# jayHuggie/PathTracer_CUDA_Interactive

Measured on AMD Instinct MI355X. Metric: Msamples/sec (rays x spp x bounces = intersect() calls per second), scenes/cbox/cbox.xml 640x480 spp=64, higher is better.
Workload: dtype f32

## Files before the change

pathtracer_cuda_interactive_amd/csrc/pt_api.hip:

```cpp
#include <cmath>
#include <cstdio>
#include <cstdlib>
#include <cstring>
#include <initializer_list>
#include <iterator>
#include <limits>
#include <mutex>
#include <type_traits>

#include "pt_scene.h"
#include "pt_transform.h"
#include "pt_denoise.h"
#include "pt_gradient.h"
#include "pt_temporal.h"
#include "pt_kernels.h"
#include "pt_kernel_q.h"
#include "pt_query.h"

using namespace ptk;

static thread_local std::string g_err;
int pt_fail(int code, const std::string& msg) { g_err = msg; return code; }
static int fail(int code, const std::string& msg) { return pt_fail(code, msg); }

// ... 84 lines not shown
    bool lds_scene() const { return res == 1 || res == 2; }
};

int choose_trace(const pt_scene* S, int traversal, bool nee, bool listed, TraceChoice* out) {
    TraceChoice c{};
    c.which = which_tree(S);
    c.res = scene_residency(S, c.which);
    const bool exact = traversal == PT_TRAVERSAL_EXACT;
    if (nee && (S->opt_kernel < 2 || !exact))
        return fail(PT_ERR_UNSUPPORTED, "PT_RENDER_NEE runs on the default kernel with exact traversal only");
    c.family = S->opt_kernel == 1 ? 1 : (S->opt_kernel == 3 && !nee && exact && !listed) ? 3 : 2;
    c.prune = !exact; c.stats = S->opt_stats != 0; c.nee = nee; c.list = listed;
    c.postpone = c.family == 3 && !c.lds_scene() && c.which == 1;
    c.spec = !(S->tri_only && S->opt_specialize) ? 0 : (S->diffuse_only ? 2 : 1);
    if (nee && c.spec == 1) c.spec = 0;
    if (c.family == 2)
        c.sched = v2_schedule((nee || listed) ? V2Schedule{0, 0, 6} : V2Schedule{(int)S->opt_v2_thresh, (int)S->opt_v2_inner, (int)S->opt_v2_minw},
                              c.lds_scene(), c.which == 1 && !nee);
    const pt_scene::Tree& T = S->tree[c.which];
    c.reg_stack = S->opt_reg_stack && c.family == 2 && !nee && !listed && c.spec == 2 && !S->opt_v2_thresh && !S->opt_v2_inner &&
                  (c.sched.minw == 5 || c.sched.minw == 6) &&
                  reg_stack_on(c.res, c.sched.thresh, c.sched.inner, c.which == 1, T.stack_cap - 1, T.num_nodes, S->dev.num_prims);
    c.sweep = S->opt_leaf_sweep && leaf_sweep_on(c.reg_stack, exact, c.stats, c.res, S->dev.num_prims, (int)S->sweep.count) &&
              S->sweep_tab.p && sweep_layout_fits(S->sweep.count, (uint32_t)S->dev.num_prims, (uint32_t)T.num_nodes, kLdsNodeStride);
    c.block_threads = c.family == 3 ? kQBlock : kBlock;
    c.feed_waves = c.family == 3 ? kQS : kBlock / 64;
    c.redo_lanes = c.family == 3 ? kQS * 64 : kBlock;
    *out = c;
    return PT_OK;
}

LdsPlan make_plan(const pt_scene* S, const TraceChoice& c) {
    LdsPlan lp{};
    const pt_scene::Tree& T = S->tree[c.which];
    uint32_t off = 0;
    if (c.res == 3) {
        const uint32_t stack_bytes = (uint32_t)(kBlock / 64) * (uint32_t)T.stack_cap * 64u * 4u;
        const uint32_t budget = S->opt_lds_budget_kb > 0 ? (uint32_t)S->opt_lds_budget_kb * 1024u : kTopLdsBudget;
        const uint32_t room = budget > stack_bytes ? budget - stack_bytes : 0u;
        lp.top_count = std::min<uint32_t>(T.top_avail, room / (uint32_t)sizeof(DNode));
        lp.nodes_off = 0;
        off = lp.top_count * (uint32_t)sizeof(DNode);
    } else if (c.res != 0) {
        lp.nodes_off = off;
        off = align16(off + (c.res == 2 ? 8u * oct_table_pitch((uint32_t)T.num_nodes, kLdsNodeStride)
                                        : (uint32_t)T.num_nodes * kLdsNodeStride));
        lp.prims_off = off; off = align16(off + (uint32_t)S->dev.num_prims * sizeof(DPrim));
// ... 122 lines not shown
        if (kV2Schedules[k].thresh == c.sched.thresh && kV2Schedules[k].inner == c.sched.inner && kV2Schedules[k].minw == c.sched.minw) si = k;
    return among<0, 1, 2, 3, 4, 5, 6, 7, 8>(si, [&](auto SI) { return among<0, 1, 2, 3>(c.res, [&](auto R) {
           return among<false, true>(c.nee, [&](auto N) { return among<false, true>(c.list, [&](auto LI) {
           static constexpr V2Schedule s = kV2Schedules[PT_CONST(SI)];
           if constexpr (!v2_compiled(PT_CONST(R), false, s, 0, PT_CONST(N), PT_CONST(LI))) return TraceEntry{};
           else return among<0, 1, 2>(c.spec, [&](auto SP) { return among<false, true>(c.prune, [&](auto P) {
           return among<false, true>(c.stats, [&](auto S) {
               if constexpr (v2_compiled(PT_CONST(R), PT_CONST(P), s, PT_CONST(SP), PT_CONST(N), PT_CONST(LI)))
                   return v2k<PT_CONST(R), PT_CONST(P), PT_CONST(S), s.thresh, s.inner, s.minw, PT_CONST(SP), PT_CONST(N), PT_CONST(LI)>();
               else return TraceEntry{}; }); }); }); }); }); }); });
}
#undef PT_CONST

void launch_trace(const pt_scene* S, const TraceChoice& c, const TraceEntry& e, int grid, hipStream_t stream, const RenderDev& rd,
                  const LdsPlan& lp, const QParams& qp, float4* samples) {
    void* const fn = const_cast<void*>(e.fn);
    if (c.family == 3)
        hipLaunchKernelGGL(reinterpret_cast<TraceFnQ>(fn), dim3(grid), dim3(c.block_threads), lp.total, stream, S->dev, rd, lp, qp,
                           samples, S->work_counter(), S->counters());
    else if (c.sweep) {
        const SweepClasses cls = S->sweep_classes_now();
        hipLaunchKernelGGL(reinterpret_cast<SweepFn>(fn), dim3(grid), dim3(c.block_threads), lp.total, stream, S->dev, rd, lp,
                           samples, S->work_counter(), S->counters(),
                           SweepLayoutDev{S->sweep_tab_now(), S->sweep.count, sweep_classes_pitch(cls), cls.pairs, cls.fam});
    } else
        hipLaunchKernelGGL(reinterpret_cast<TraceFn>(fn), dim3(grid), dim3(c.block_threads), lp.total, stream, S->dev, rd, lp,
                           samples, S->work_counter(), S->counters());
}

int read_slot_sums(const pt_scene* S, unsigned long long* out) {
    std::vector<unsigned long long> raw(kTimelineBase);
    HIP_TRY(hipMemcpy(raw.data(), S->counters(), raw.size() * sizeof(unsigned long long), hipMemcpyDeviceToHost));
    std::fill(out, out + kSlotStride, 0ull);
    for (int s = 0; s < kCounterSlots; s++)
        for (int k = 0; k < kSlotStride; k++) out[k] += raw[(size_t)s * kSlotStride + k];
    return PT_OK;
}

int launch_grid(int num_cus, int blocks_per_cu, uint64_t work_items, int block_threads = kBlock) {
    const uint64_t blocks_needed = (work_items + (uint64_t)block_threads - 1) / (uint64_t)block_threads;
    return (int)std::max<uint64_t>(1, std::min<uint64_t>((uint64_t)num_cus * (uint64_t)blocks_per_cu, blocks_needed));
}

struct RowSel {
    int begin, step, count;
};

// ... 1193 lines not shown
    else if (k == "lds_budget_kb") S->opt_lds_budget_kb = value;
    else if (k == "chunk") S->opt_chunk = value;
    else if (k == "item_order") S->opt_item_order = value;
    else if (k == "specialize") S->opt_specialize = value;
    else if (k == "timing_frames") {
        if (value < 0 || value > 4096) return fail(PT_ERR_INVALID_ARG, "timing_frames must be 0 .. 4096");
        S->opt_timing_frames = value;
    }
    else if (k == "kernel") { if (value < 1 || value > 3) return fail(PT_ERR_INVALID_ARG, "kernel must be 1, 2 or 3"); S->opt_kernel = value; }
    else if (k == "frames_in_flight") {
        if (value < 1 || value > kMaxFramesInFlight) return fail(PT_ERR_INVALID_ARG, "frames_in_flight must be 1 .. " + std::to_string(kMaxFramesInFlight));
        S->opt_frames_in_flight = value;
    }
    else if (k == "q_target") S->opt_q_target = value;
    else if (k == "q_swap") S->opt_q_swap = value;
    else if (k == "q_low") S->opt_q_low = value;
    else if (k == "v2_thresh") S->opt_v2_thresh = value;
    else if (k == "v2_inner") S->opt_v2_inner = value;
    else if (k == "v2_minw") S->opt_v2_minw = value;
    else if (k == "reg_stack") { if (value != 0 && value != 1) return fail(PT_ERR_INVALID_ARG, "reg_stack must be 0 or 1"); S->opt_reg_stack = value; }
    else if (k == "leaf_sweep") { if (value != 0 && value != 1) return fail(PT_ERR_INVALID_ARG, "leaf_sweep must be 0 or 1"); S->opt_leaf_sweep = value; }
    else if (k == "sweep_pairs") { if (value != 0 && value != 1) return fail(PT_ERR_INVALID_ARG, "sweep_pairs must be 0 or 1"); S->opt_sweep_pairs = value; }
    else if (k == "sweep_families") { if (value != 0 && value != 1) return fail(PT_ERR_INVALID_ARG, "sweep_families must be 0 or 1"); S->opt_sweep_families = value; }
    else if (k == "query_refill") { if (value < 0 || value > 64) return fail(PT_ERR_INVALID_ARG, "query_refill must be 0 (automatic) .. 64"); S->opt_query_refill = value; }
    else if (k == "query_guides") { if (value < 0 || value > 2) return fail(PT_ERR_INVALID_ARG, "query_guides must be 0 (automatic), 1 or 2"); S->opt_query_guides = value; }
    else if (k == "query_blocks") { if (value < 0 || value > 4096) return fail(PT_ERR_INVALID_ARG, "query_blocks must be 0 (automatic) .. 4096"); S->opt_query_blocks = value; }
    else if (k == "tree_cost" || k == "rebuild_at_permille") {
        if (k == "tree_cost" && value != 0 && value != 1) return fail(PT_ERR_INVALID_ARG, "tree_cost must be 0 or 1");
        if (k == "rebuild_at_permille" && value != 0 && value < 1001) return fail(PT_ERR_INVALID_ARG, "rebuild_at_permille must be 0 (never) or at least 1001");
        const bool was_on = S->cost_on();
        (k == "tree_cost" ? S->opt_tree_cost : S->opt_rebuild_at) = value;
        if (!was_on && S->cost_on()) S->cost_forget();
    }
    else return fail(PT_ERR_INVALID_ARG, "unknown option " + k);
    return PT_OK;
}

int pt_scene_get_info(pt_scene* S, const char* key, int64_t* value) {
    if (!S || !key || !value) return fail(PT_ERR_INVALID_ARG, "null argument");
    const std::string k(key);
    TraceChoice next;
    (void)choose_trace(S, k == "vgprs_pruned" ? PT_TRAVERSAL_PRUNED : PT_TRAVERSAL_EXACT, false, false, &next);
    DeviceGuard guard;
    unsigned long long c[kSlotStride];
    if (k == "grid") *value = S->info_grid;
    else if (k == "lds_bytes") *value = S->info_lds_bytes;
// ... 42 lines not shown
        const int t = k[9] - '0';
        *value = (S->cost_on() && (t == 0 || S->have_fast)) ? cost_permille(S, t) : 1000;
    }
    else if (k == "refit_shape0" || k == "refit_shape1") {
        const ptf::Plan& pl = S->refit_plan[k[11] - '0'];
        *value = !pl.built ? 0 : pl.whole_tree ? 1 : pl.narrow_top < pl.levels - 1 ? 2 : 3;
    }
    else if (k == "kernel") *value = S->info_kernel;
    else if (k == "trace_variant") *value = S->info_trace_variant;
    else if (k == "path_bank") *value = S->info_path_bank;
    else if (k == "leaf_sweep") *value = S->info_leaf_sweep;
    else if (k == "sweep_boxes") *value = S->sweep_groups;
    else if (k.rfind("sweep_share_pairs", 0) == 0 || k.rfind("sweep_flat_pairs", 0) == 0 || k == "sweep_general_pairs") {
        const SweepClasses c = S->sweep_classes_now();
        const bool flat = k[6] == 'f';
        const std::string axis = k.substr(flat ? 16 : 17);
        if (k == "sweep_general_pairs") *value = c.pairs.general;
        else if (axis.empty()) *value = sweep_classes_sharing(c, flat, -1);
        else if (axis == "_x" || axis == "_y" || axis == "_z") *value = sweep_classes_sharing(c, flat, axis[1] - 'x');
        else return fail(PT_ERR_INVALID_ARG, "unknown info key " + k);
    }
    else if (k == "sweep_pair2_records") *value = sweep_pair2_records(S->sweep_classes_now().fam);
    else if (k == "sweep_valu_model") *value = sweep_valu_model(S->sweep_classes_now());
    else if (k == "reg_stack") *value = S->info_reg_stack;
    else if (k == "block_threads") *value = S->info_kernel == 3 ? kQBlock : kBlock;
    else if (k == "frames_in_flight") *value = S->opt_frames_in_flight;
    else if (k == "query_chunk") *value = ptq::kQueryChunk;
    else if (k == "query_guides") *value = S->info_query_guides;
    else if (k == "query_grid") *value = S->info_query_grid;
    else if (k.rfind("qdiag", 0) == 0 && k.size() >= 6 && k.size() <= 7 && k.find_first_not_of("0123456789", 5) == std::string::npos &&
             std::stoi(k.substr(5)) < 11) {
        int rc = synced_slot_sums(S, guard, c);
        if (rc) return rc;
        *value = (int64_t)c[4 + std::stoi(k.substr(5))];
    }
    else if (k.rfind("diag", 0) == 0 && k.size() >= 5 && k.size() <= 7 && k.find_first_not_of("0123456789", 4) == std::string::npos &&
             std::stoi(k.substr(4)) < 8 + kNumCounters - kTimelineBase) {
        unsigned long long v = 0;
        const int idx = std::stoi(k.substr(4));
        if (idx < 8) {
            int rc = synced_slot_sums(S, guard, c);
            if (rc) return rc;
            v = c[4 + idx];
        } else {
            if (int grc = guard.enter(S->device)) return grc;
            HIP_TRY(hipStreamSynchronize(S->last_stream));
// ... 113 lines not shown
```

pathtracer_cuda_interactive_amd/csrc/pt_kernels.h:

```cpp
#pragma once

#include <hip/hip_runtime.h>

#include <type_traits>

#include "pt_layout.h"
#include "pt_leaf_sweep.h"
#include "pt_math.h"
#include "pt_path_bank.h"
#include "pt_path_index.h"
#include "pt_sweep_layout.h"
#include "pt_sweep_families.h"
#include "pt_sweep_pairs.h"
#include "pt_temporal.h"
#include "pt_trace.h"

namespace ptk {

using namespace ptl;


#ifndef PT_BLOCK
#define PT_BLOCK 256
#endif
constexpr int kBlock = PT_BLOCK;
constexpr uint32_t kMaxChunk = 256;

__device__ __forceinline__ uint32_t lane_rank(unsigned long long mask) {
    return __builtin_amdgcn_mbcnt_hi((uint32_t)(mask >> 32), __builtin_amdgcn_mbcnt_lo((uint32_t)mask, 0u));
}

__device__ __forceinline__ unsigned long long wave_sum(unsigned long long v) {
    for (int off = 32; off > 0; off >>= 1) v += __shfl_down(v, off, 64);
    return v;
}
// ... 251 lines not shown

template <int RES, bool PRUNE, bool STATS, int MINW>
__global__ __launch_bounds__(kBlock, (kBlock > 256 ? 1 : MINW)) void trace_kernel_v2_reg(SceneDev scn, RenderDev rp, LdsPlan lp,
                                                              float4* __restrict__ samples,
                                                              uint32_t* __restrict__ work_counter,
                                                              unsigned long long* __restrict__ counters) {
    constexpr int THRESH = 40, INNER = 162, SPEC = 2;
    constexpr bool NEE = false, LIST = false, REG = true;
#include "pt_trace_v2_body.h"
}

#ifndef PT_SWEEP_LEAF_STEPS
#define PT_SWEEP_LEAF_STEPS 4
#endif
#ifndef PT_SWEEP_THRESH
#define PT_SWEEP_THRESH 48
#endif
struct SweepLayoutDev {
    const unsigned char* tab;
    uint32_t groups;
    uint32_t box_pitch;
    SweepPairClasses classes;
    SweepFamilyClasses fam;
};
struct SweepKernelArgs {
    SceneDev scn; RenderDev rp; LdsPlan lp; float4* samples; uint32_t* work_counter; unsigned long long* counters; SweepLayoutDev sweep;
};
static_assert(offsetof(SweepKernelArgs, rp) == offsetof(TraceKernelArgs, rp), "reload_render_args reads rp at TraceKernelArgs' offset");
static_assert(offsetof(SweepLayoutDev, fam) + 16 <= sizeof(SweepLayoutDev), "step (3) reads the three PAIR2 count words as one load of four: the fourth must lie inside the argument");

__device__ __forceinline__ ptd::SceneView make_sweep_view(const SceneDev& scn, const LdsPlan& lp, const SweepLayoutDev& sweep,
                                                          unsigned char* smem) {
    const uint32_t slots_off = sweep_slots_off(sweep.groups);
    stage_to_lds(smem + lp.nodes_off, sweep.tab, slots_off);
    const DPrim* gslots = reinterpret_cast<const DPrim*>(sweep.tab + slots_off);
    DPrim* lslots = reinterpret_cast<DPrim*>(smem + lp.nodes_off + slots_off);
    for (uint32_t i = threadIdx.x; i < (uint32_t)scn.num_prims; i += blockDim.x) {
        const float4 a = ptd::ld4(gslots + i, 0), b = ptd::ld4(gslots + i, 1), c = ptd::ld4(gslots + i, 2);
        DPrim g;
        g.v[0] = a.x; g.v[1] = a.y; g.v[2] = a.z; g.v[3] = a.w; g.v[4] = b.x; g.v[5] = b.y; g.v[6] = b.z; g.v[7] = b.w; g.v[8] = c.x;
        g.info = __builtin_bit_cast(int32_t, c.y); g.light = __builtin_bit_cast(int32_t, c.z); g.pad = __builtin_bit_cast(int32_t, c.w);
        const DPrim r = sweep_stage_record(g);
        float4* d = reinterpret_cast<float4*>(lslots + i);
        d[0] = make_float4(r.v[0], r.v[1], r.v[2], r.v[3]);
        d[1] = make_float4(r.v[4], r.v[5], r.v[6], r.v[7]);
        d[2] = make_float4(r.v[8], c.y, c.z, c.w);
    }
    stage_to_lds(smem + lp.prims_off, scn.prims, (uint32_t)scn.num_prims * sizeof(DPrim));
    stage_to_lds(smem + lp.normals_off, scn.normals, (uint32_t)scn.num_prims * sizeof(DNormals));
    stage_to_lds(smem + lp.mats_off, scn.materials, (uint32_t)scn.num_materials * sizeof(DMaterial));
    stage_to_lds(smem + lp.emis_off, scn.emission, (uint32_t)scn.num_emission * sizeof(DEmission));
    __syncthreads();
    ptd::SceneView sv;
    sv.top_nodes = nullptr;
    sv.top_count = 0;
    sv.nodes = reinterpret_cast<const DNode*>(smem + lp.nodes_off);
    sv.prims = reinterpret_cast<const DPrim*>(smem + lp.prims_off);
    sv.normals = reinterpret_cast<const DNormals*>(smem + lp.normals_off);
    sv.materials = reinterpret_cast<const DMaterial*>(smem + lp.mats_off);
    sv.emission = reinterpret_cast<const DEmission*>(smem + lp.emis_off);
    sv.node_stride = kLdsNodeStride;
    sv.oct_stride = sweep.box_pitch;
    sv.lights = scn.lights;
    sv.num_emission = scn.num_emission;
    sv.root_ref = scn.root_ref;
    sv.fixed_order = scn.fixed_order;
    sv.ref_nodes = scn.ref_nodes; sv.ref_path = scn.ref_path; sv.ref_anc = scn.ref_anc; sv.ref_levels = scn.ref_levels;
    sv.bg = ptm::mk(scn.bg[0], scn.bg[1], scn.bg[2]);
    return sv;
}
// ... 399 lines not shown
```

pathtracer_cuda_interactive_amd/csrc/pt_scene.h:

```cpp
#pragma once
#include <hip/hip_runtime.h>

#include <algorithm>
#include <chrono>
#include <cstdint>
#include <string>
#include <utility>
#include <vector>

#include "../../include/pt_api.h"
#include "pt_internal.h"
#include "pt_layout.h"
#include "pt_leaf_sweep.h"
#include "pt_sweep_families.h"
#include "pt_sweep_pairs.h"
#include "pt_scene_refit.h"

#define HIP_TRY(expr)                                                                              \
    do {                                                                                           \
        hipError_t e_ = (expr);                                                                    \
        if (e_ != hipSuccess)                                                                      \
            return pt_fail(e_ == hipErrorNoDevice ? PT_ERR_NO_DEVICE : PT_ERR_DEVICE,              \
                           std::string(#expr) + ": " + hipGetErrorString(e_));                     \
    } while (0)

#define ENTER_DEVICE(S) DeviceGuard guard; if (int grc_ = guard.enter((S)->device)) return grc_

namespace ptkc {
constexpr int kBlock = 256, kCounterStride = 32, kQueryRing = 64, kLdsNodeStride = 64;
}

using namespace ptl;

template <class T>
struct DevBuf {
    T* p = nullptr;
    size_t n = 0;
// ... 176 lines not shown
    int64_t opt_top_cache = 1;
    int64_t opt_fast_tree = 1;
    int64_t opt_chunk = 0;
    int64_t opt_lds_budget_kb = 0;
    int64_t opt_item_order = 1;
    int64_t opt_xcd_regions = 0;
    int64_t opt_kernel = 2;
    int64_t opt_q_target = 0, opt_q_swap = 0, opt_q_low = 0;
    int64_t opt_v2_thresh = 0, opt_v2_inner = 0, opt_v2_minw = 0;
    int64_t opt_reg_stack = 1;
    int64_t opt_leaf_sweep = 1;
    int64_t opt_sweep_pairs = 1;
    int64_t opt_sweep_families = 1;
    SweepTable sweep{};
    int sweep_groups = 0;
    DevBuf<unsigned char> sweep_tab;
    DevBuf<unsigned char> sweep_tab_pairs[2];
    SweepClasses sweep_classes[2] = {};
    SweepClasses sweep_classes_now() const {
        if (!sweep.count) return SweepClasses{};
        return opt_sweep_pairs && sweep_tab_pairs[opt_sweep_families].p ? sweep_classes[opt_sweep_families] : sweep_classes_of_pairs(sweep_pairs_none(sweep.count));
    }
    const unsigned char* sweep_tab_now() const { return opt_sweep_pairs && sweep_tab_pairs[opt_sweep_families].p ? sweep_tab_pairs[opt_sweep_families].p : sweep_tab.p; }
    int64_t create_us[7] = {0, 0, 0, 0, 0, 0, 0}, sweep_on_device = 0;
    int64_t info_grid = 0, info_lds_bytes = 0, info_lds_scene = 0, info_passes = 0, info_occupancy = 0, info_blocks_per_cu = 0, info_debug_reruns = 0, fast_cost_permille = 0, info_kernel = 0, info_trace_variant = 0, info_path_bank = 0, info_reg_stack = 0, info_leaf_sweep = 0;
    struct PassEvents { hipEvent_t t0, t1, r0, r1; };
    struct FrameRec { std::vector<PassEvents> ev; size_t passes = 0; };
    std::vector<FrameRec> frames;
    uint64_t frame_seq = 0;
    int64_t opt_timing_frames = 1;
    const FrameRec* last_frame() const { return frame_seq && !frames.empty() ? &frames[(frame_seq - 1) % frames.size()] : nullptr; }
    void drop_events() {
        for (auto& f : frames)
            for (auto& pe : f.ev) { (void)hipEventDestroy(pe.t0); (void)hipEventDestroy(pe.t1); (void)hipEventDestroy(pe.r0); (void)hipEventDestroy(pe.r1); }
        frames.clear();
        frame_seq = 0;
    }
    const void* cfg_fn = nullptr;
    uint32_t cfg_lds = 0;
    int cfg_occ = 0;
    ~pt_scene() {
        drop_query();
        for (auto& T : tree) { T.nodes.release(); T.nodes_oct.release(); }
        drop_slots(); drop_events();
        prims.release(); normals.release(); materials.release(); emission.release(); lights.release();
        for (auto& pl : refit_plan) ptf::plan_release(&pl);
// ... 31 lines not shown
```

pathtracer_cuda_interactive_amd/csrc/pt_scene_life.hip:

```cpp
#include <cmath>
#include <cstdlib>
#include <cstring>
#include <exception>
#include <limits>
#include <queue>

#include "pt_scene.h"
#include "pt_tree_sweep.h"
#include "pt_sweep_build.h"
#include "pt_scene_prep.h"
#include "pt_tree_cost.h"
#include "pt_scene_transform.h"
#include "pt_transform.h"
#include "pt_sweep_layout.h"
#include "pt_sweep_families.h"
#include "pt_sweep_pairs.h"

namespace {
using namespace ptkc;

constexpr uint32_t kOctNodeLimit = 24 * 1024;
constexpr int kMaxStack = 64;
constexpr int kMinInternalTree = 16;
constexpr int kDeviceSweepMin = 4096;
#ifndef PT_TOP_NODES
#define PT_TOP_NODES 512
#endif
constexpr uint32_t kTopNodes = PT_TOP_NODES;
constexpr uint32_t kMaxLdsBudget = 160 * 1024;

bool prepared_on_device(int N) {
    const char* v = std::getenv("PT_SWEEP_BUILD");
    return N >= kDeviceSweepMin && !(v && std::string(v) == "host");
}

struct TreeHost {
    std::vector<DNode> nodes;
    int32_t root_ref = 0;
// ... 270 lines not shown
    int32_t froot = 0, fdepth = 0;
    bool ok = true, fnested = true;
    try {
        pts::build_sweep_tree(boxes_host, N, fnodes, &froot, &fdepth);
    } catch (const std::exception&) {
        ok = false;
    }
    built(try_device);
    c.ok = ok && convert_tree(fnodes.data(), (int)fnodes.size(), froot, N, c.host, nullptr, &fnested, true) == PT_OK && fnested;
    return c;
}

void drop_internal_tree(pt_scene* S, const char* why) {
    S->have_fast = S->fast_is_callers_topology = false;
    S->no_fast_why = why;
    S->tree[1].nodes.release(); S->tree[1].nodes_oct.release(); S->tree[1].have_oct = false;
    S->ref_path.release(); S->ref_anc.release();
}

int64_t probe_permille(const unsigned long long v[2]) { return v[0] ? (int64_t)((1000ull * v[1] + v[0] / 2) / v[0]) : 1000; }
bool probe_wins(const unsigned long long v[2]) { return v[1] * 100ull < v[0] * 90ull; }

int make_sweep_tables(const TreeHost& fast, const DPrim* prims, int N, SweepTable& sweep, int& sweep_groups, DevBuf<unsigned char>& sweep_tab,
                      DevBuf<unsigned char> (&sweep_tab_pairs)[2], SweepClasses (&classes)[2]) {
    sweep = SweepTable{};
    sweep_groups = 0;
    for (SweepClasses& c : classes) c = SweepClasses{};
    SweepGroup groups[kSweepMaxPrims];
    const int n = build_sweep_groups(fast.nodes.data(), (int)fast.nodes.size(), N, kLdsNodeStride, groups);
    if (n > 0) {
        sweep_groups = n;
        std::vector<unsigned char> tab(n <= kSweepMaxBoxes ? sweep_layout_bytes((uint32_t)n, (uint32_t)N) : 0);
        SweepGroup paired[kSweepMaxBoxes];
        int perm[kSweepMaxBoxes];
        SweepClasses cls[2] = {};
        std::vector<unsigned char> tab_pairs[2];
        const DNode* nodes = fast.nodes.data();
        const int num_nodes = (int)fast.nodes.size();
        bool ok = n <= kSweepMaxBoxes && build_sweep_layout(groups, n, nodes, num_nodes, kLdsNodeStride, prims, N, tab.data());
        for (int m = 0; ok && m < 2; m++) {
            tab_pairs[m].resize(tab.size());
            ok = build_sweep_families(groups, n, nodes, num_nodes, kLdsNodeStride, m, paired, perm, &cls[m]) &&
                 build_sweep_layout(paired, n, nodes, num_nodes, kLdsNodeStride, prims, N, tab_pairs[m].data()) &&
                 build_sweep_family_tables(paired, n, cls[m], nodes, num_nodes, kLdsNodeStride, tab_pairs[m].data());
        }
        if (ok && !(sweep_stream_fits(sweep_classes_of_pairs(sweep_pairs_none((uint32_t)n)), (uint32_t)n, (uint32_t)N) &&
                    sweep_stream_fits(cls[0], (uint32_t)n, (uint32_t)N) && sweep_stream_fits(cls[1], (uint32_t)n, (uint32_t)N)))
            return pt_fail(PT_ERR_UNSUPPORTED, "sweep tables: the record stream would read past the staged sweep region");
        if (ok) {
            if (int rc = sweep_tab.ensure(tab.size())) return rc;
            HIP_TRY(hipMemcpy(sweep_tab.p, tab.data(), tab.size(), hipMemcpyHostToDevice));
            for (int m = 0; m < 2; m++) {
                if (int rc = sweep_tab_pairs[m].ensure(tab_pairs[m].size())) return rc;
                HIP_TRY(hipMemcpy(sweep_tab_pairs[m].p, tab_pairs[m].data(), tab_pairs[m].size(), hipMemcpyHostToDevice));
                classes[m] = cls[m];
            }
            sweep.count = (uint32_t)n;
            std::copy(groups, groups + n, sweep.g);
        }
    }
    return PT_OK;
}

int check_desc(const pt_scene_desc* d) {
    if (!d) return pt_fail(PT_ERR_INVALID_ARG, "null scene description");
    if (d->num_shapes <= 0 || !d->shapes) return pt_fail(PT_ERR_BAD_SCENE, "scene has no shapes");
    if (d->num_nodes != 2 * d->num_shapes - 1 || !d->nodes)
        return pt_fail(PT_ERR_BAD_SCENE, "BVH must have 2*num_shapes-1 nodes (bvh.cu:16-54)");
    if (d->root < 0 || d->root >= d->num_nodes) return pt_fail(PT_ERR_BAD_SCENE, "BVH root out of range");
    if (d->num_materials <= 0 || !d->materials) return pt_fail(PT_ERR_BAD_SCENE, "scene has no materials");
    if (d->num_meshes < 0 || (d->num_meshes > 0 && !d->meshes)) return pt_fail(PT_ERR_BAD_SCENE, "bad mesh array");
    if (d->num_lights < 0 || (d->num_lights > 0 && !d->lights)) return pt_fail(PT_ERR_BAD_SCENE, "bad light array");
    if (int rc = check_materials(d)) return rc;
    return check_meshes(d, d->num_materials);
}

struct CreateState {
    bool on_device = false, nested = true;
    std::vector<DPrim> prims; std::vector<DNormals> normals;
// ... 139 lines not shown
    S->diffuse_only = all_diffuse(d);
    S->create_us[1] = clock.lap();
    if ((rc = callers_tree(d, S, c))) return rc;
    S->create_us[2] = clock.lap();
    if (N < kMinInternalTree) {
        S->no_fast_why = "fewer than 16 shapes";
    } else if (!c.nested) {
        S->no_fast_why = "the caller's boxes do not nest";
    } else {
        c.cand = internal_tree(c.boxes_dev.p, c.on_device ? nullptr : c.boxes_host.data(), N,
                               [&](bool again) { if (!again) S->create_us[3] = clock.lap(); });
        if (!c.cand.ok) S->no_fast_why = "the internal tree could not be built";
    }
    S->sweep_on_device = c.cand.on_device ? 1 : 0;
    c.boxes_dev.release();
    std::vector<float>().swap(c.boxes_host);
    S->create_us[4] = clock.lap();
    if ((rc = upload_scene(d, S, c))) return rc;
    if ((rc = probe_and_decide(d, S, c.ref_inner))) return rc;
    S->create_us[5] = clock.lap();
    if ((rc = tie_tables(d, S, c))) return rc;
    S->sweep = SweepTable{}; S->sweep_groups = 0;
    if (S->have_fast && !c.cand.on_device && !S->fast_is_callers_topology && N <= kSweepMaxPrims &&
        (rc = make_sweep_tables(c.cand.host, c.prims.data(), N, S->sweep, S->sweep_groups, S->sweep_tab, S->sweep_tab_pairs, S->sweep_classes)))
        return rc;
    HIP_TRY(hipDeviceSynchronize());
    S->create_us[6] = clock.lap(); S->create_us[0] = clock.total();
    select_tree(S, 0);
    S->scene_bytes = (uint32_t)std::min<size_t>(
        c.ref_inner * sizeof(DNode) + (size_t)N * (sizeof(DPrim) + sizeof(DNormals)) + (size_t)d->num_materials * sizeof(DMaterial) +
            (size_t)std::max(d->num_lights, 1) * sizeof(DEmission) + 64, 0xffffffffu);
    return PT_OK;
}

int ensure_staging(pt_scene* S) {
    const size_t N = (size_t)S->dev.num_prims;
    int rc;
    if ((rc = S->st_prims.ensure(N)) || (rc = S->prev_prims.ensure(N)) || (rc = S->st_normals.ensure(N))) return rc;
    return S->st_status.ensure(1);
}

int ensure_cost(pt_scene* S) {
    int rc;
    const size_t need = std::max(ptc::partials_needed(S->tree[0].num_nodes), ptc::partials_needed(S->tree[1].num_nodes));
    if ((rc = S->cost_partials.ensure(need)) || (rc = S->cost_dev.ensure(4))) return rc;
    if (!S->cost_host) HIP_TRY(hipHostMalloc(reinterpret_cast<void**>(&S->cost_host), 4 * sizeof(double), hipHostMallocDefault));
    return PT_OK;
// ... 42 lines not shown
    unsigned int bad = 0;
    if (!whole || n_trees == 0) {
        if ((rc = S->st_boxes.ensure((size_t)N * 6)) || (rc = ptf::leaf_boxes(S->st_prims.p, N, S->st_boxes.p, S->st_status.p))) return rc;
        HIP_TRY(hipMemcpy(&bad, S->st_status.p, sizeof bad, hipMemcpyDeviceToHost));
    }
    for (int t = 0; t < n_trees && !bad; t++) {
        pt_scene::Tree& T = S->tree[t];
        if ((rc = ptf::refit_tree(S->refit_plan[t], T.nodes.p, T.have_oct ? T.nodes_oct.p : nullptr, T.num_nodes, S->st_prims.p,
                                  whole ? nullptr : S->st_boxes.p, N, S->st_status.p)))
            return rc;
    }
    if (whole && n_trees) HIP_TRY(hipMemcpy(&bad, S->st_status.p, sizeof bad, hipMemcpyDeviceToHost));
    if (bad) return pt_fail(PT_ERR_UNSUPPORTED, std::string(who) + ": a new coordinate, radius or leaf box is not finite");
    for (int t = 0; costs && t < n_trees; t++) S->cost_pending_now[t] = enqueue_cost(S, S->tree[t], 2 + t) == PT_OK;
    S->prev_prims.swap(S->st_prims);
    S->prims.swap(S->prev_prims);
    S->have_prev = true;
    S->normals.swap(S->st_normals);
    S->dev.prims = S->prims.p; S->dev.normals = S->normals.p;
    S->tri_only = tri_only;
    S->sweep_groups = 0; S->sweep.count = 0;
    S->sweep_tab.release();
    for (int m = 0; m < 2; m++) { S->sweep_tab_pairs[m].release(); S->sweep_classes[m] = SweepClasses{}; }
    *us_refit = clock.lap();
    return PT_OK;
}

int rebuild_scene(pt_scene* S) {
    if (!S->have_fast)
        return pt_fail(PT_ERR_UNSUPPORTED, std::string("pt_scene_rebuild: the handle holds no tie tables, pt_scene_create kept no internal tree: ") +
                                               (S->no_fast_why[0] ? S->no_fast_why : "none was built"));
    const int N = S->dev.num_prims;
    const pt_scene::Tree& T0 = S->tree[0];
    StageClock clock;
    int64_t us[4] = {0, 0, 0, 0};
    int rc;
    DevBuf<float> boxes_dev;
    if ((rc = boxes_dev.ensure((size_t)N * 6)) || (rc = ptf::tree_leaf_boxes(T0.nodes.p, T0.num_nodes, N, boxes_dev.p))) return rc;
    InternalTree cand = internal_tree(boxes_dev.p, nullptr, N, [&](bool again) { if (again) clock.rewind(); us[1] = clock.lap(); });
    if (cand.copy_error != hipSuccess)
        return pt_fail(cand.copy_error == hipErrorNoDevice ? PT_ERR_NO_DEVICE : PT_ERR_DEVICE, std::string("hipMemcpy(leaf_boxes.data(), boxes_dev.p, leaf_boxes.size() * sizeof(float), hipMemcpyDeviceToHost): ") + hipGetErrorString(cand.copy_error));
    if (!cand.ok)
        return pt_fail(PT_ERR_UNSUPPORTED, "pt_scene_rebuild: no internal tree could be built of the leaf boxes (not finite, or they no longer nest)");
    if (!cand.on_device && (rc = upload_tree(cand.tree, cand.host))) return rc;
    boxes_dev.release();
    SceneDev d0 = S->dev, d1 = S->dev;
    tree_view(S, d0, 0, false);
    tree_view(S, d1, cand.tree, 1, false);
    for (SceneDev* dv : {&d0, &d1}) { dv->ref_path = nullptr; dv->ref_anc = nullptr; dv->ref_levels = 0; dv->redo_stack = nullptr; }
    unsigned long long v[2] = {0, 0};
    if ((rc = probe_trees(d0, d1, v))) return rc;
    const bool adopt = probe_wins(v);
    us[2] = clock.lap();
    ptf::Plan plan;
    SweepTable sweep{}; int sweep_groups = 0; DevBuf<unsigned char> sweep_tab, sweep_tab_pairs[2]; SweepClasses sweep_classes[2] = {};
    double cost = 0.0;
    if (adopt) {
        if (S->refit_plan[1].built && (rc = ptf::plan_build(cand.tree.nodes.p, cand.tree.num_nodes, N, &plan))) return rc;
        struct PlanGuard { ptf::Plan* p; ~PlanGuard() { if (p) ptf::plan_release(p); } } plan_guard{&plan};
        if (!cand.on_device && N <= kSweepMaxPrims) {
            std::vector<DPrim> prims((size_t)N);
            HIP_TRY(hipMemcpy(prims.data(), S->prims.p, prims.size() * sizeof(DPrim), hipMemcpyDeviceToHost));
            if ((rc = make_sweep_tables(cand.host, prims.data(), N, sweep, sweep_groups, sweep_tab, sweep_tab_pairs, sweep_classes))) return rc;
        }
        if (S->cost_on()) {
            if ((rc = ensure_cost(S)) || (rc = enqueue_cost(S, cand.tree, 3))) return rc;
            HIP_TRY(hipStreamSynchronize(nullptr));
            cost = S->cost_host[3];
        }
        std::swap(S->tree[1], cand.tree);
        S->have_fast = true; S->fast_is_callers_topology = false;
        S->fast_cost_permille = probe_permille(v);
        S->sweep_on_device = cand.on_device ? 1 : 0;
        std::swap(S->refit_plan[1], plan);
        plan_guard.p = &plan;
        S->sweep = sweep; S->sweep_groups = sweep_groups;
        S->sweep_tab.swap(sweep_tab);
        for (int m = 0; m < 2; m++) { S->sweep_tab_pairs[m].swap(sweep_tab_pairs[m]); S->sweep_classes[m] = sweep_classes[m]; }
        S->cfg_fn = S->q_cfg_fn = nullptr;
        if (S->cost_on()) { S->cost_ref[1] = S->cost_now[1] = cost; S->cost_have_ref[1] = true; }
    } else if (S->cost_on() && S->cost_have_ref[1] && S->cost_now[1] > 0.0) {
        S->cost_ref[1] = S->cost_now[1];
    }
    us[3] = clock.lap();
    us[0] = clock.total();
    select_tree(S, 0);
    S->rebuilds++; S->rebuild_adopted = adopt ? 1 : 0; S->rebuild_cost_permille = probe_permille(v);
    std::copy(us, us + 4, S->rebuild_us);
    return PT_OK;
}

void rebuild_by_policy(pt_scene* S) {
    if (S->opt_rebuild_at <= 0 || !S->have_fast || !S->cost_pending_now[1]) return;
    if (hipStreamSynchronize(nullptr) != hipSuccess) return;
    collect_costs(S);
    if (cost_permille(S, 1) < S->opt_rebuild_at) return;
    if (rebuild_scene(S) == PT_OK) S->rebuilds_auto++;
}

int update_scene(pt_scene* S, const pt_scene_desc* d, int flags) {
    const bool geometry = (flags & PT_UPDATE_GEOMETRY) != 0, shading = (flags & PT_UPDATE_SHADING) != 0;
// ... 216 lines not shown
```

pathtracer_cuda_interactive_amd/csrc/pt_trace_sweep_body.h:

```cpp
    extern __shared__ __attribute__((aligned(16))) unsigned char smem[];
    constexpr int THRESH = PT_SWEEP_THRESH;
    typedef const __attribute__((address_space(3))) unsigned char* LdsBytes;
    typedef float f2v __attribute__((ext_vector_type(2)));
    typedef const __attribute__((address_space(3))) f2v* LdsF2;
    const uint32_t n_groups = sweep.groups;
    const uint32_t box_pitch = sweep.box_pitch;
    const uint64_t cls_bits = __builtin_bit_cast(uint64_t, sweep.classes);
    const ptd::SceneView sv = make_sweep_view(scn, lp, sweep, smem);
    const ptd::lds_f4v* slots = (const ptd::lds_f4v*)(smem + lp.nodes_off + sweep_slots_off(n_groups));

    const int lane = threadIdx.x & 63;
    const int wave = threadIdx.x >> 6;

    WorkFeed feed;
    feed_init(feed, rp);
    PathBank bank;
    bank_init(bank);
    float bank_dx = 0.0f, bank_dy = 0.0f, bank_dz = 0.0f;
    uint32_t bank_lo = 0, bank_hi = 0;
    uint32_t bank_w = 0, bank_inc_lo = 0, bank_inc_hi = 0;
    bool alive = false;
    ptd::Ray ray;
    ray.org = ptm::mk(0, 0, 0); ray.dir = ptm::mk(0, 0, 1); ray.tnear = 0; ray.tfar = 0;
    ptd::Trav tv;
// ... 22 lines not shown
        const int n_pend = __popcll(__ballot(idle && (alive || work_left)));
        if (n_pend >= THRESH || idle_mask == ~0ull) {
            if (n_pend == 0) break;
            if (idle && alive && tv.redo) {
                ptd::TravStats st_redo;
                st_redo.nodes = 0; st_redo.leaves = 0;
                ray.tfar = depth == 0 ? __builtin_inff() : FLT_MAX;
                tv.best = ptd::intersect<false, false>(sv_ref, ray, redo_stk, st_redo);
                tv.redo = false;
            }
            if (idle && alive) {
                bool cont = false;
                if (tv.best.prim < 0) {
                    L = L + T * sv.bg;
                } else {
                    const ptd::Surface sf = ptd::make_surface<true>(sv, ray, tv.best);
                    cont = ptd::shade_and_bounce<true, false>(sv, sf, ray, rng, L, T, depth, rp.rr_depth, nullptr);
                    depth++;
                    if (depth >= rp.max_depth) cont = false;
                }
                if (!cont) {
                    samples[my_w] = make_float4(L.x, L.y, L.z, 0.0f);
                    alive = false;
                }
            }
            unsigned long long want = __ballot(idle && !alive);
#pragma nounroll
            for (int round = 0; round < 2 && want; round++) {
                if (bank.left == 0) {
                    feed_reserve(feed, rp, work_counter, lane);
                    if (feed.cur >= feed.end) break;
                    bank_fill(bank, feed.cur, feed.end);
                    const RenderDev rg = reload_render_args<false>();
                    const PathStart ps = start_path<false>(rg, feed.region, bank_item(feed.cur, (uint32_t)lane));
                    bank_dx = ps.ray.dir.x; bank_dy = ps.ray.dir.y; bank_dz = ps.ray.dir.z;
                    bank_lo = (uint32_t)ps.rng.state; bank_hi = (uint32_t)(ps.rng.state >> 32);
                    const BankIndex bi = bank_index_pack(ps.sample_index, ps.rng.inc);
                    bank_w = bi.sample_index; bank_inc_lo = bi.inc_lo; bank_inc_hi = bi.inc_hi;
                }
                uint32_t first;
                const uint32_t k = bank_take(bank, (uint32_t)__popcll(want), first);
                const uint32_t rank = lane_rank(want);
                const bool take = idle && !alive && rank < k;
                const int src = take ? (int)(first + rank) : lane;
                const float dx = __shfl(bank_dx, src, 64), dy = __shfl(bank_dy, src, 64), dz = __shfl(bank_dz, src, 64);
                const uint32_t lo = __shfl(bank_lo, src, 64), hi = __shfl(bank_hi, src, 64);
// ... 66 lines not shown
                    bx = sweep_shared_pairs<1, false>(bx, win, cls.share[1], o, inv, h);
                    bx = sweep_shared_pairs<2, false>(bx, win, cls.share[2], o, inv, h);
#pragma clang loop vectorize(disable) interleave(disable) unroll(disable)
                    for (uint32_t k = cls.general; k != 0; k--) {
                        const f2v b1 = bx[4], b2 = bx[5];
                        __builtin_amdgcn_sched_barrier(0);
                        const float d_anx = win.p0.x - o.x, d_any = win.p0.y - o.y, d_anz = win.p1.x - o.z;
                        const float d_afx = win.p1.y - o.x, d_afy = win.p2.x - o.y, d_afz = win.p2.y - o.z;
                        const float d_bnx = win.p3.x - o.x, d_bny = win.p3.y - o.y, d_bnz = b1.x - o.z;
                        const float d_bfx = b1.y - o.x, d_bfy = b2.x - o.y, d_bfz = b2.y - o.z;
                        bx = sweep_window_read(win, bx, 6);
                        const float tna = ptm::fmax2(0.0f, ptm::fmax2(ptm::fmax2(d_anx * inv.x, d_any * inv.y), d_anz * inv.z));
                        const float tfa = ptm::fmin2(ptm::fmin2(d_afx * inv.x, d_afy * inv.y), d_afz * inv.z);
                        const float tnb = ptm::fmax2(0.0f, ptm::fmax2(ptm::fmax2(d_bnx * inv.x, d_bny * inv.y), d_bnz * inv.z));
                        const float tfb = ptm::fmin2(ptm::fmin2(d_bfx * inv.x, d_bfy * inv.y), d_bfz * inv.z);
                        sweep_shift_in_two(h, tfa, tna, tfb, tnb);
                    }
                    if (cls.single) {
                        const float tn = ptm::fmax2(ptm::fmax2((win.p0.x - o.x) * inv.x, (win.p0.y - o.y) * inv.y), (win.p1.x - o.z) * inv.z);
                        const float tf = ptm::fmin2(ptm::fmin2((win.p1.y - o.x) * inv.x, (win.p2.x - o.y) * inv.y), (win.p2.y - o.z) * inv.z);
                        const float tn0 = ptm::fmax2(0.0f, tn);
                        asm("v_cmp_ge_f32_e32 vcc, %1, %2\n\ts_nop 1\n\tv_addc_co_u32_e32 %0, vcc, %0, %0, vcc" : "+v"(h) : "v"(tf), "v"(tn0) : "vcc");
                    }
                    hits = sweep_hits_align(h, n_groups);
                }
            }
        }
#pragma unroll
        for (int k = 0; k < N_LEAF; k++) {
            if ((hits | pend) != 0u) {
                uint32_t slot = pend;
                if (pend == 0u) {
                    slot = sweep_first_group(hits);
                    hits = sweep_clear_group(hits, slot);
                }
                pend = ptd::leaf_test_slot(sv, slots, ray, tv, slot);
            }
        }
    }
    flush_counters<false>(counters, lane, lane == 0 ? n_paths : 0u, lane == 0 ? n_segs : 0u, st);
```

Measured before the change: 47110.

## Skip leaf tests of coplanar sweep groups containing the ray origin's surface

Builds a per-primitive skip table holding an axis, a plane coordinate and a bitmask of sweep groups that lie flat on that same axis-aligned plane. The table is staged into LDS next to the sweep layout. After a bounce, if the new ray origin lies exactly on the hit primitive's plane, those coplanar groups are masked out of the next sweep's hit set, so their leaf triangle tests are skipped. This suits Cornell-box-style scenes with flat walls. In exchange it adds an LDS read and a compare per bounce, extra LDS space, and host-side table construction, and it relies on exact float equality between the origin and the plane coordinate.

```diff
diff --git a/pathtracer_cuda_interactive_amd/csrc/pt_api.hip b/pathtracer_cuda_interactive_amd/csrc/pt_api.hip
--- a/pathtracer_cuda_interactive_amd/csrc/pt_api.hip
+++ b/pathtracer_cuda_interactive_amd/csrc/pt_api.hip
@@ -130,7 +130,8 @@
                   (c.sched.minw == 5 || c.sched.minw == 6) &&
                   reg_stack_on(c.res, c.sched.thresh, c.sched.inner, c.which == 1, T.stack_cap - 1, T.num_nodes, S->dev.num_prims);
     c.sweep = S->opt_leaf_sweep && leaf_sweep_on(c.reg_stack, exact, c.stats, c.res, S->dev.num_prims, (int)S->sweep.count) &&
-              S->sweep_tab.p && sweep_layout_fits(S->sweep.count, (uint32_t)S->dev.num_prims, (uint32_t)T.num_nodes, kLdsNodeStride);
+              S->sweep_tab.p && sweep_layout_fits(S->sweep.count, (uint32_t)S->dev.num_prims, (uint32_t)T.num_nodes, kLdsNodeStride) &&
+              S->sweep_skip.p && sweep_skip_fits(S->sweep.count, (uint32_t)S->dev.num_prims, (uint32_t)T.num_nodes, kLdsNodeStride);
     c.block_threads = c.family == 3 ? kQBlock : kBlock;
     c.feed_waves = c.family == 3 ? kQS : kBlock / 64;
     c.redo_lanes = c.family == 3 ? kQS * 64 : kBlock;
@@ -299,7 +300,7 @@
         const SweepClasses cls = S->sweep_classes_now();
         hipLaunchKernelGGL(reinterpret_cast<SweepFn>(fn), dim3(grid), dim3(c.block_threads), lp.total, stream, S->dev, rd, lp,
                            samples, S->work_counter(), S->counters(),
-                           SweepLayoutDev{S->sweep_tab_now(), S->sweep.count, sweep_classes_pitch(cls), cls.pairs, cls.fam});
+                           SweepLayoutDev{S->sweep_tab_now(), S->sweep.count, sweep_classes_pitch(cls), cls.pairs, cls.fam, S->sweep_skip_now()});
     } else
         hipLaunchKernelGGL(reinterpret_cast<TraceFn>(fn), dim3(grid), dim3(c.block_threads), lp.total, stream, S->dev, rd, lp,
                            samples, S->work_counter(), S->counters());
@@ -1539,6 +1540,7 @@
     else if (k == "leaf_sweep") { if (value != 0 && value != 1) return fail(PT_ERR_INVALID_ARG, "leaf_sweep must be 0 or 1"); S->opt_leaf_sweep = value; }
     else if (k == "sweep_pairs") { if (value != 0 && value != 1) return fail(PT_ERR_INVALID_ARG, "sweep_pairs must be 0 or 1"); S->opt_sweep_pairs = value; }
     else if (k == "sweep_families") { if (value != 0 && value != 1) return fail(PT_ERR_INVALID_ARG, "sweep_families must be 0 or 1"); S->opt_sweep_families = value; }
+    else if (k == "sweep_self_skip") { if (value != 0 && value != 1) return fail(PT_ERR_INVALID_ARG, "sweep_self_skip must be 0 or 1"); S->opt_sweep_self_skip = value; }
     else if (k == "query_refill") { if (value < 0 || value > 64) return fail(PT_ERR_INVALID_ARG, "query_refill must be 0 (automatic) .. 64"); S->opt_query_refill = value; }
     else if (k == "query_guides") { if (value < 0 || value > 2) return fail(PT_ERR_INVALID_ARG, "query_guides must be 0 (automatic), 1 or 2"); S->opt_query_guides = value; }
     else if (k == "query_blocks") { if (value < 0 || value > 4096) return fail(PT_ERR_INVALID_ARG, "query_blocks must be 0 (automatic) .. 4096"); S->opt_query_blocks = value; }
@@ -1627,6 +1629,8 @@
     }
     else if (k == "sweep_pair2_records") *value = sweep_pair2_records(S->sweep_classes_now().fam);
     else if (k == "sweep_valu_model") *value = sweep_valu_model(S->sweep_classes_now());
+    else if (k == "sweep_skip_groups") *value = S->sweep_skip_info_now().groups;
+    else if (k == "sweep_skip_planes") *value = S->sweep_skip_info_now().planes;
     else if (k == "reg_stack") *value = S->info_reg_stack;
     else if (k == "block_threads") *value = S->info_kernel == 3 ? kQBlock : kBlock;
     else if (k == "frames_in_flight") *value = S->opt_frames_in_flight;
diff --git a/pathtracer_cuda_interactive_amd/csrc/pt_kernels.h b/pathtracer_cuda_interactive_amd/csrc/pt_kernels.h
--- a/pathtracer_cuda_interactive_amd/csrc/pt_kernels.h
+++ b/pathtracer_cuda_interactive_amd/csrc/pt_kernels.h
@@ -11,6 +11,7 @@
 #include "pt_path_index.h"
 #include "pt_sweep_layout.h"
 #include "pt_sweep_families.h"
+#include "pt_sweep_skip.h"
 #include "pt_sweep_pairs.h"
 #include "pt_temporal.h"
 #include "pt_trace.h"
@@ -308,6 +309,7 @@
     uint32_t box_pitch;
     SweepPairClasses classes;
     SweepFamilyClasses fam;
+    const unsigned char* skip;
 };
 struct SweepKernelArgs {
     SceneDev scn; RenderDev rp; LdsPlan lp; float4* samples; uint32_t* work_counter; unsigned long long* counters; SweepLayoutDev sweep;
@@ -332,6 +334,7 @@
         d[1] = make_float4(r.v[4], r.v[5], r.v[6], r.v[7]);
         d[2] = make_float4(r.v[8], c.y, c.z, c.w);
     }
+    stage_to_lds(smem + lp.nodes_off + sweep_skip_off(sweep.groups, (uint32_t)scn.num_prims), sweep.skip, sweep_skip_bytes((uint32_t)scn.num_prims));
     stage_to_lds(smem + lp.prims_off, scn.prims, (uint32_t)scn.num_prims * sizeof(DPrim));
     stage_to_lds(smem + lp.normals_off, scn.normals, (uint32_t)scn.num_prims * sizeof(DNormals));
     stage_to_lds(smem + lp.mats_off, scn.materials, (uint32_t)scn.num_materials * sizeof(DMaterial));
diff --git a/pathtracer_cuda_interactive_amd/csrc/pt_scene.h b/pathtracer_cuda_interactive_amd/csrc/pt_scene.h
--- a/pathtracer_cuda_interactive_amd/csrc/pt_scene.h
+++ b/pathtracer_cuda_interactive_amd/csrc/pt_scene.h
@@ -13,6 +13,7 @@
 #include "pt_layout.h"
 #include "pt_leaf_sweep.h"
 #include "pt_sweep_families.h"
+#include "pt_sweep_skip.h"
 #include "pt_sweep_pairs.h"
 #include "pt_scene_refit.h"
 
@@ -235,6 +236,12 @@
         return opt_sweep_pairs && sweep_tab_pairs[opt_sweep_families].p ? sweep_classes[opt_sweep_families] : sweep_classes_of_pairs(sweep_pairs_none(sweep.count));
     }
     const unsigned char* sweep_tab_now() const { return opt_sweep_pairs && sweep_tab_pairs[opt_sweep_families].p ? sweep_tab_pairs[opt_sweep_families].p : sweep_tab.p; }
+    DevBuf<unsigned char> sweep_skip;
+    SweepSkipInfo sweep_skip_info[3] = {};
+    int64_t opt_sweep_self_skip = 1;
+    int sweep_skip_index() const { return !opt_sweep_self_skip ? 0 : opt_sweep_pairs && sweep_tab_pairs[opt_sweep_families].p ? 2 + (int)opt_sweep_families : 1; }
+    const unsigned char* sweep_skip_now() const { return sweep_skip.p ? sweep_skip.p + (size_t)sweep_skip_index() * kSweepSkipTableBytes : nullptr; }
+    SweepSkipInfo sweep_skip_info_now() const { return sweep.count && sweep_skip.p && sweep_skip_index() ? sweep_skip_info[sweep_skip_index() - 1] : SweepSkipInfo{0, 0}; }
     int64_t create_us[7] = {0, 0, 0, 0, 0, 0, 0}, sweep_on_device = 0;
     int64_t info_grid = 0, info_lds_bytes = 0, info_lds_scene = 0, info_passes = 0, info_occupancy = 0, info_blocks_per_cu = 0, info_debug_reruns = 0, fast_cost_permille = 0, info_kernel = 0, info_trace_variant = 0, info_path_bank = 0, info_reg_stack = 0, info_leaf_sweep = 0;
     struct PassEvents { hipEvent_t t0, t1, r0, r1; };
diff --git a/pathtracer_cuda_interactive_amd/csrc/pt_scene_life.hip b/pathtracer_cuda_interactive_amd/csrc/pt_scene_life.hip
--- a/pathtracer_cuda_interactive_amd/csrc/pt_scene_life.hip
+++ b/pathtracer_cuda_interactive_amd/csrc/pt_scene_life.hip
@@ -14,6 +14,7 @@
 #include "pt_transform.h"
 #include "pt_sweep_layout.h"
 #include "pt_sweep_families.h"
+#include "pt_sweep_skip.h"
 #include "pt_sweep_pairs.h"
 
 namespace {
@@ -330,10 +331,12 @@
 bool probe_wins(const unsigned long long v[2]) { return v[1] * 100ull < v[0] * 90ull; }
 
 int make_sweep_tables(const TreeHost& fast, const DPrim* prims, int N, SweepTable& sweep, int& sweep_groups, DevBuf<unsigned char>& sweep_tab,
-                      DevBuf<unsigned char> (&sweep_tab_pairs)[2], SweepClasses (&classes)[2]) {
+                      DevBuf<unsigned char> (&sweep_tab_pairs)[2], SweepClasses (&classes)[2], DevBuf<unsigned char>& sweep_skip,
+                      SweepSkipInfo (&skip_info)[3]) {
     sweep = SweepTable{};
     sweep_groups = 0;
     for (SweepClasses& c : classes) c = SweepClasses{};
+    for (SweepSkipInfo& i : skip_info) i = SweepSkipInfo{0, 0};
     SweepGroup groups[kSweepMaxPrims];
     const int n = build_sweep_groups(fast.nodes.data(), (int)fast.nodes.size(), N, kLdsNodeStride, groups);
     if (n > 0) {
@@ -343,14 +346,18 @@
         int perm[kSweepMaxBoxes];
         SweepClasses cls[2] = {};
         std::vector<unsigned char> tab_pairs[2];
+        std::vector<unsigned char> skip(4 * (size_t)kSweepSkipTableBytes, 0);
+        SweepSkipInfo si[3] = {};
         const DNode* nodes = fast.nodes.data();
         const int num_nodes = (int)fast.nodes.size();
-        bool ok = n <= kSweepMaxBoxes && build_sweep_layout(groups, n, nodes, num_nodes, kLdsNodeStride, prims, N, tab.data());
+        bool ok = n <= kSweepMaxBoxes && build_sweep_layout(groups, n, nodes, num_nodes, kLdsNodeStride, prims, N, tab.data()) &&
+                  build_sweep_skip(groups, n, nodes, num_nodes, kLdsNodeStride, prims, N, skip.data() + kSweepSkipTableBytes, &si[0]);
         for (int m = 0; ok && m < 2; m++) {
             tab_pairs[m].resize(tab.size());
             ok = build_sweep_families(groups, n, nodes, num_nodes, kLdsNodeStride, m, paired, perm, &cls[m]) &&
                  build_sweep_layout(paired, n, nodes, num_nodes, kLdsNodeStride, prims, N, tab_pairs[m].data()) &&
-                 build_sweep_family_tables(paired, n, cls[m], nodes, num_nodes, kLdsNodeStride, tab_pairs[m].data());
+                 build_sweep_family_tables(paired, n, cls[m], nodes, num_nodes, kLdsNodeStride, tab_pairs[m].data()) &&
+                 build_sweep_skip(paired, n, nodes, num_nodes, kLdsNodeStride, prims, N, skip.data() + (2 + m) * (size_t)kSweepSkipTableBytes, &si[1 + m]);
         }
         if (ok && !(sweep_stream_fits(sweep_classes_of_pairs(sweep_pairs_none((uint32_t)n)), (uint32_t)n, (uint32_t)N) &&
                     sweep_stream_fits(cls[0], (uint32_t)n, (uint32_t)N) && sweep_stream_fits(cls[1], (uint32_t)n, (uint32_t)N)))
@@ -363,6 +370,9 @@
                 HIP_TRY(hipMemcpy(sweep_tab_pairs[m].p, tab_pairs[m].data(), tab_pairs[m].size(), hipMemcpyHostToDevice));
                 classes[m] = cls[m];
             }
+            if (int rc = sweep_skip.ensure(skip.size())) return rc;
+            HIP_TRY(hipMemcpy(sweep_skip.p, skip.data(), skip.size(), hipMemcpyHostToDevice));
+            std::copy(si, si + 3, skip_info);
             sweep.count = (uint32_t)n;
             std::copy(groups, groups + n, sweep.g);
         }
@@ -548,7 +558,7 @@
     if ((rc = tie_tables(d, S, c))) return rc;
     S->sweep = SweepTable{}; S->sweep_groups = 0;
     if (S->have_fast && !c.cand.on_device && !S->fast_is_callers_topology && N <= kSweepMaxPrims &&
-        (rc = make_sweep_tables(c.cand.host, c.prims.data(), N, S->sweep, S->sweep_groups, S->sweep_tab, S->sweep_tab_pairs, S->sweep_classes)))
+        (rc = make_sweep_tables(c.cand.host, c.prims.data(), N, S->sweep, S->sweep_groups, S->sweep_tab, S->sweep_tab_pairs, S->sweep_classes, S->sweep_skip, S->sweep_skip_info)))
         return rc;
     HIP_TRY(hipDeviceSynchronize());
     S->create_us[6] = clock.lap(); S->create_us[0] = clock.total();
@@ -637,6 +647,8 @@
     S->sweep_groups = 0; S->sweep.count = 0;
     S->sweep_tab.release();
     for (int m = 0; m < 2; m++) { S->sweep_tab_pairs[m].release(); S->sweep_classes[m] = SweepClasses{}; }
+    S->sweep_skip.release();
+    for (SweepSkipInfo& i : S->sweep_skip_info) i = SweepSkipInfo{0, 0};
     *us_refit = clock.lap();
     return PT_OK;
 }
@@ -668,7 +680,7 @@
     const bool adopt = probe_wins(v);
     us[2] = clock.lap();
     ptf::Plan plan;
-    SweepTable sweep{}; int sweep_groups = 0; DevBuf<unsigned char> sweep_tab, sweep_tab_pairs[2]; SweepClasses sweep_classes[2] = {};
+    SweepTable sweep{}; int sweep_groups = 0; DevBuf<unsigned char> sweep_tab, sweep_tab_pairs[2], sweep_skip; SweepClasses sweep_classes[2] = {}; SweepSkipInfo sweep_skip_info[3] = {};
     double cost = 0.0;
     if (adopt) {
         if (S->refit_plan[1].built && (rc = ptf::plan_build(cand.tree.nodes.p, cand.tree.num_nodes, N, &plan))) return rc;
@@ -676,7 +688,7 @@
         if (!cand.on_device && N <= kSweepMaxPrims) {
             std::vector<DPrim> prims((size_t)N);
             HIP_TRY(hipMemcpy(prims.data(), S->prims.p, prims.size() * sizeof(DPrim), hipMemcpyDeviceToHost));
-            if ((rc = make_sweep_tables(cand.host, prims.data(), N, sweep, sweep_groups, sweep_tab, sweep_tab_pairs, sweep_classes))) return rc;
+            if ((rc = make_sweep_tables(cand.host, prims.data(), N, sweep, sweep_groups, sweep_tab, sweep_tab_pairs, sweep_classes, sweep_skip, sweep_skip_info))) return rc;
         }
         if (S->cost_on()) {
             if ((rc = ensure_cost(S)) || (rc = enqueue_cost(S, cand.tree, 3))) return rc;
@@ -692,6 +704,8 @@
         S->sweep = sweep; S->sweep_groups = sweep_groups;
         S->sweep_tab.swap(sweep_tab);
         for (int m = 0; m < 2; m++) { S->sweep_tab_pairs[m].swap(sweep_tab_pairs[m]); S->sweep_classes[m] = sweep_classes[m]; }
+        S->sweep_skip.swap(sweep_skip);
+        std::copy(sweep_skip_info, sweep_skip_info + 3, S->sweep_skip_info);
         S->cfg_fn = S->q_cfg_fn = nullptr;
         if (S->cost_on()) { S->cost_ref[1] = S->cost_now[1] = cost; S->cost_have_ref[1] = true; }
     } else if (S->cost_on() && S->cost_have_ref[1] && S->cost_now[1] > 0.0) {
diff --git a/pathtracer_cuda_interactive_amd/csrc/pt_sweep_skip.h b/pathtracer_cuda_interactive_amd/csrc/pt_sweep_skip.h
--- /dev/null
+++ b/pathtracer_cuda_interactive_amd/csrc/pt_sweep_skip.h
@@ -0,0 +1,99 @@
+#pragma once
+#include <stdint.h>
+#include <string.h>
+
+#include "pt_sweep_layout.h"
+
+namespace ptl {
+
+constexpr int kSweepSelfSkipOff = 0, kSweepSelfSkipOn = 1;
+
+struct SweepSkipEntry {
+    float c;
+    uint32_t mask;
+    uint32_t axis;
+};
+static_assert(sizeof(SweepSkipEntry) == 12, "12 bytes per primitive");
+
+PT_SWEEP_HD uint32_t sweep_skip_bytes(uint32_t num_prims) { return (num_prims * (uint32_t)sizeof(SweepSkipEntry) + 15u) & ~15u; }
+constexpr uint32_t kSweepSkipTableBytes = kSweepMaxPrims * (uint32_t)sizeof(SweepSkipEntry);
+static_assert(kSweepSkipTableBytes % 16u == 0, "sweep_skip_bytes(kSweepMaxPrims) is the table");
+PT_SWEEP_HD uint32_t sweep_skip_off(uint32_t groups, uint32_t num_prims) { return sweep_layout_bytes(groups, num_prims); }
+PT_SWEEP_HD bool sweep_skip_fits(uint32_t groups, uint32_t num_prims, uint32_t num_nodes, uint32_t node_stride) {
+    return sweep_skip_off(groups, num_prims) + sweep_skip_bytes(num_prims) <= 8u * oct_table_pitch(num_nodes, node_stride);
+}
+
+struct SweepSkipInfo {
+    uint32_t groups;
+    uint32_t planes;
+};
+
+inline int sweep_group_flat_axis(const SweepGroup& g, const DNode* nodes, int num_nodes, uint32_t node_stride, const DPrim* prims,
+                                 int num_prims, float* c) {
+    const uint32_t node = g.box_off / node_stride, rest = g.box_off % node_stride;
+    if (node >= (uint32_t)num_nodes || (rest != 0 && rest != kSweepBoxBytes)) return -1;
+    const float* box = rest ? nodes[node].rmin : nodes[node].lmin;
+    for (int a = 0; a < 3; a++) {
+        if (!(box[a] == box[3 + a])) continue;
+        bool on_plane = true;
+        for (uint64_t m = sweep_group_mask(g); m && on_plane; m = sweep_clear_lowest(m)) {
+            const int32_t prim = sweep_lowest(m);
+            if (prim >= num_prims || prims[prim].info < 0) { on_plane = false; break; }
+            for (int v = 0; v < 3; v++) on_plane = on_plane && prims[prim].v[3 * v + a] == box[a];
+        }
+        if (on_plane) { *c = box[a]; return a; }
+    }
+    return -1;
+}
+
+inline bool sweep_group_on_plane(const SweepGroup& g, int axis, float c, const DNode* nodes, int num_nodes, uint32_t node_stride,
+                                 const DPrim* prims, int num_prims) {
+    const uint32_t node = g.box_off / node_stride, rest = g.box_off % node_stride;
+    if (node >= (uint32_t)num_nodes || (rest != 0 && rest != kSweepBoxBytes)) return false;
+    const float* box = rest ? nodes[node].rmin : nodes[node].lmin;
+    if (!(box[axis] == c && box[3 + axis] == c)) return false;
+    for (uint64_t m = sweep_group_mask(g); m; m = sweep_clear_lowest(m)) {
+        const int32_t prim = sweep_lowest(m);
+        if (prim >= num_prims || prims[prim].info < 0) return false;
+        for (int v = 0; v < 3; v++)
+            if (!(prims[prim].v[3 * v + axis] == c)) return false;
+    }
+    return true;
+}
+
+inline bool build_sweep_skip(const SweepGroup* groups, int count, const DNode* nodes, int num_nodes, uint32_t node_stride, const DPrim* prims,
+                             int num_prims, unsigned char* out, SweepSkipInfo* info) {
+    if (count < 1 || count > kSweepMaxBoxes || num_prims < count || num_prims > kSweepMaxPrims || num_nodes < 1) return false;
+    memset(out, 0, kSweepSkipTableBytes);
+    SweepSkipInfo si{0, 0};
+    for (int k = 0; k < count; k++) {
+        float c = 0.0f;
+        const int axis = sweep_group_flat_axis(groups[k], nodes, num_nodes, node_stride, prims, num_prims, &c);
+        if (axis < 0) continue;
+        uint32_t mask = 0;
+        for (int j = 0; j < count; j++)
+            if (j == k || sweep_group_on_plane(groups[j], axis, c, nodes, num_nodes, node_stride, prims, num_prims)) mask |= 0x80000000u >> j;
+        si.groups++;
+        bool first = true;
+        for (int j = 0; j < k && first; j++) {
+            float cj = 0.0f;
+            if (sweep_group_flat_axis(groups[j], nodes, num_nodes, node_stride, prims, num_prims, &cj) == axis && cj == c) first = false;
+        }
+        if (first) si.planes++;
+        const SweepSkipEntry e{c, mask, (uint32_t)axis};
+        for (uint64_t m = sweep_group_mask(groups[k]); m; m = sweep_clear_lowest(m)) {
+            const int32_t prim = sweep_lowest(m);
+            if (prim >= num_prims) return false;
+            memcpy(out + (size_t)prim * sizeof(SweepSkipEntry), &e, sizeof(e));
+        }
+    }
+    if (info) *info = si;
+    return true;
+}
+
+PT_SWEEP_HD uint32_t sweep_skip_word(const SweepSkipEntry& e, const float org[3]) {
+    const float oa = e.axis == 0u ? org[0] : e.axis == 1u ? org[1] : org[2];
+    return oa == e.c ? e.mask : 0u;
+}
+
+}
diff --git a/pathtracer_cuda_interactive_amd/csrc/pt_trace_sweep_body.h b/pathtracer_cuda_interactive_amd/csrc/pt_trace_sweep_body.h
--- a/pathtracer_cuda_interactive_amd/csrc/pt_trace_sweep_body.h
+++ b/pathtracer_cuda_interactive_amd/csrc/pt_trace_sweep_body.h
@@ -68,6 +68,14 @@
                 if (!cont) {
                     samples[my_w] = make_float4(L.x, L.y, L.z, 0.0f);
                     alive = false;
+                } else {
+                    typedef const __attribute__((address_space(3))) uint32_t* LdsWords;
+                    LdsWords e = (LdsWords)((LdsBytes)smem + lp.nodes_off + sweep_skip_off(n_groups, (uint32_t)scn.num_prims) +
+                                            (uint32_t)tv.best.prim * (uint32_t)sizeof(SweepSkipEntry));
+                    const float skip_c = __builtin_bit_cast(float, e[0]);
+                    const uint32_t skip_mask = e[1], skip_axis = e[2];
+                    const float oa = skip_axis == 0u ? ray.org.x : skip_axis == 1u ? ray.org.y : ray.org.z;
+                    hits = oa == skip_c ? skip_mask : 0u;
                 }
             }
             unsigned long long want = __ballot(idle && !alive);
@@ -180,7 +188,9 @@
                         const float tn0 = ptm::fmax2(0.0f, tn);
                         asm("v_cmp_ge_f32_e32 vcc, %1, %2\n\ts_nop 1\n\tv_addc_co_u32_e32 %0, vcc, %0, %0, vcc" : "+v"(h) : "v"(tf), "v"(tn0) : "vcc");
                     }
-                    hits = sweep_hits_align(h, n_groups);
+                    hits = sweep_hits_align(h, n_groups) & ~hits;
+                } else {
+                    hits = 0u;
                 }
             }
         }
```

After: 48920 (median of 6 runs). +3.9%, better.
